# khalil-research/CaVE

Measured on NVIDIA B200. Metric: cave_loss_grad_instances_per_sec, higher is better.
Workload: dtype f64

## Files before the change

cave_b200/build.py:

```python
from __future__ import annotations

import os
import shutil
import subprocess

HERE = os.path.dirname(os.path.abspath(__file__))
CSRC = os.path.join(HERE, "csrc")
OUT_DIR = os.path.join(HERE, "_C")
LIB = os.path.join(OUT_DIR, "libcave_b200.so")
SOURCES = ["scan_kernel.cu", "solve_kernel.cu", "solve_inst_f32_f32.cu", "solve_inst_f32_f64.cu",
           "solve_inst_f64_f32.cu", "solve_inst_f64_f64.cu", "gram_kernel.cu", "dense_solve.cu", "tsp_dp.cu", "abi.cu"]
HEADERS = ["ctx.cuh", "layout.cuh", "dense.cuh", "scan_kernel.cuh", "solve_kernel.cuh", "solve_kernel_impl.cuh", "solver_core.cuh",
           os.path.join("..", "..", "include", "cave_b200.h")]
NVCC_FLAGS = ["-gencode", "arch=compute_100a,code=sm_100a", "-lineinfo", "-O3", "-std=c++17",
              "-Xcompiler", "-fPIC", "-Xptxas", "-v"]


PER_FILE_FLAGS = {"dense_solve.cu": ["-rdc=true", "-maxrregcount=128"]}


def _nvcc() -> str:
    nvcc = shutil.which("nvcc") or "/usr/local/cuda/bin/nvcc"
    if not os.path.exists(nvcc):
        raise RuntimeError("nvcc not found; cannot build the CUDA library")
    return nvcc


def is_fresh() -> bool:
    if not os.path.exists(LIB):
        return False
    t = os.path.getmtime(LIB)
    deps = [os.path.join(CSRC, s) for s in SOURCES + HEADERS] + [os.path.abspath(__file__)]
    return all(os.path.getmtime(p) <= t for p in deps)


def build(force: bool = False, verbose: bool = False, alt_name: str | None = None) -> str:
    if alt_name is None and not force and is_fresh():
        return LIB
    os.makedirs(OUT_DIR, exist_ok=True)
    objs, logs = [], []
    procs = []
    for s in SOURCES:
        obj = os.path.join(OUT_DIR, s.replace(".cu", ".o") if alt_name is None else s.replace(".cu", ".alt.o"))
        cmd = [_nvcc(), *NVCC_FLAGS, *PER_FILE_FLAGS.get(s, []), *os.environ.get("CAVE_NVCC_EXTRA", "").split(),
               "-c", os.path.join(CSRC, s), "-o", obj]
        procs.append((s, subprocess.Popen(cmd, stdout=subprocess.PIPE, stderr=subprocess.STDOUT, text=True)))
        objs.append(obj)
    for s, pr in procs:
        out, _ = pr.communicate()
        logs.append(f"== {s}\n{out}")
        if pr.returncode != 0:
            raise RuntimeError(f"nvcc failed on {s}:\n{out}")
    if alt_name is None:
        with open(os.path.join(OUT_DIR, "ptxas.log"), "w") as f:
            f.write("\n".join(logs))
    if verbose:
        print("\n".join(logs))
    target = LIB if alt_name is None else os.path.join(OUT_DIR, alt_name)
    subprocess.check_call([_nvcc(), "-gencode", "arch=compute_100a,code=sm_100a", "-shared", "-o", target, *objs,
                           "-lcudart_static", "-lpthread", "-ldl", "-lrt"])
    return target


if __name__ == "__main__":
    import sys
    alt = [a for a in sys.argv[1:] if a.endswith(".so")]
    print(build(force=True, verbose="-v" in sys.argv, alt_name=alt[0] if alt else None))
```

cave_b200/csrc/abi.cu:

```cuda
#include <cuda_runtime.h>
#include <stdarg.h>
#include <stdio.h>
#include <stdlib.h>
#include <string.h>
#include <atomic>
#include <string>

#include "../../include/cave_b200.h"
#include "layout.cuh"
#include "scan_kernel.cuh"
#include "solve_kernel.cuh"
#include "dense.cuh"

namespace cave {
size_t tsp_slot_floats(int n);
cudaError_t launch_tsp(const float* cost, int N, int n, int* tour, double* obj, void* scratch, int n_slots, cudaStream_t stream);
}

namespace {

thread_local std::string g_err;
std::atomic<unsigned long long> g_launches{0};

int fail(int code, const char* fmt, ...) {
// ... 225 lines not shown
    return pack_impl(A, m_rows, B, m_max, d, pack, pack_bytes, stream, (flags & 1) != 0);
}

int cave_pack_sparse(const int64_t* inst_off, const int64_t* row_ptr, const int32_t* col, const float* val, int64_t B,
                     int64_t m_max, int64_t d, int32_t flags, void* pack, size_t pack_bytes, void* stream) {
    if (!inst_off || !row_ptr || !col || !val) return fail(CAVE_EINVAL, "inst_off, row_ptr, col and val must not be null");
    SparseIn in;
    in.inst_off = (const long long*)inst_off; in.row_ptr = (const long long*)row_ptr; in.col = col; in.val = val;
    return pack_impl(nullptr, nullptr, B, m_max, d, pack, pack_bytes, stream, (flags & 1) != 0, &in);
}

int cave_warm_bytes(int64_t n_instances, int64_t m_max, int64_t d, size_t* out) {
    if (!out) return fail(CAVE_EINVAL, "out is null");
    if (int e = check_shape(n_instances, m_max, d)) return e;
    *out = (size_t)n_instances * cave::warm_slot_bytes(m_max);
    return CAVE_OK;
}

int cave_dense_warm_bytes(int64_t n_instances, int64_t m_max, int64_t d, size_t* out) {
    if (!out) return fail(CAVE_EINVAL, "out is null");
    if (int e = check_shape(n_instances, m_max, d)) return e;
    *out = (size_t)n_instances * cave::dense_warm_slot_bytes(m_max);
    return CAVE_OK;
}

static int forward_backward_impl(const float* A, const int32_t* m_rows, const void* pred, int64_t B, int64_t m_max, int64_t d,
                                 double sign, int mode, double inner_ratio, int reduction, int io_dtype, int compute_dtype,
                                 const cave_solver_opts* opts, void* loss, void* loss_i, void* grad, void* proj, void* rnorm,
                                 int32_t* status, int32_t* iters, void* pack, size_t pack_bytes, void* scratch,
                                 size_t scratch_bytes, void* warm, size_t warm_bytes, void* warm_dense,
                                 size_t warm_dense_bytes, const void* gram, size_t gram_bytes, void* stream) {
    const bool indexed = opts && opts->inst_index;
    if ((!A && !indexed) || !pred || !loss_i || !grad || !pack || !scratch) return fail(CAVE_EINVAL, "A, pred, loss_i, grad, pack, scratch must not be null");
    if (indexed && !opts->warm_pack) return fail(CAVE_EINVAL, "inst_index needs warm_pack (a pack built over the whole dataset)");
    if (indexed && opts->n_packed <= 0) return fail(CAVE_EINVAL, "n_packed must be positive with inst_index");
    if (int e = check_shape(B, m_max, d)) return e;
    if (mode < CAVE_MODE_EXACT || mode > CAVE_MODE_HEURISTIC) return fail(CAVE_EINVAL, "bad mode %d", mode);
    if (reduction < CAVE_REDUCE_MEAN || reduction > CAVE_REDUCE_NONE) return fail(CAVE_EINVAL, "bad reduction %d", reduction);
    if ((io_dtype != CAVE_F32 && io_dtype != CAVE_F64) || (compute_dtype != CAVE_F32 && compute_dtype != CAVE_F64))
        return fail(CAVE_EINVAL, "bad dtype (io %d, compute %d)", io_dtype, compute_dtype);
    if (!(sign == 1.0 || sign == -1.0)) return fail(CAVE_EINVAL, "sign must be +1 or -1");
    if (!(inner_ratio >= 0.0 && inner_ratio <= 1.0)) return fail(CAVE_EINVAL, "inner_ratio must be in [0, 1]");
    if (reduction != CAVE_REDUCE_NONE && !loss) return fail(CAVE_EINVAL, "loss must not be null for mean/sum");
    if (((uintptr_t)scratch & 255) != 0 || ((uintptr_t)pack & 255) != 0) return fail(CAVE_EINVAL, "pack and scratch must be 256-byte aligned");

    const int64_t Bpack = indexed ? opts->n_packed : B;
    if (int e = check_shape(Bpack, m_max, d)) return e;
    const cave::PackLayout PL = cave::make_pack_layout(Bpack, m_max, d);
    if (pack_bytes < PL.total) return fail(CAVE_ENOSPC, "pack buffer has %zu bytes, %zu needed", pack_bytes, PL.total);
    const ScratchPlan SPn = plan_scratch(opts, B, m_max, d);
    const size_t T = 8;
    const int64_t n_slots = SPn.n_slots;
    const cave::ScratchLayout SL = cave::make_scratch_layout(B, d, SPn.cr, SPn.cz, T, n_slots, SPn.n_large, SPn.large_bytes, SPn.small_bytes);
    const bool dense = dense_enabled(opts, A, m_max, d, mode);
    cave::DenseLayout DL;
    memset(&DL, 0, sizeof(DL));
    if (dense) DL = cave::make_dense_layout(B, m_max, d, dense_slots(opts, B, m_max, d), SL.total);
    const size_t need = dense ? DL.total : SL.total;
    if (scratch_bytes < need) return fail(CAVE_ENOSPC, "scratch buffer has %zu bytes, %zu needed", scratch_bytes, need);
    if (warm) {
        const size_t wneed = (size_t)Bpack * cave::warm_slot_bytes(m_max);
        if (warm_bytes < wneed) return fail(CAVE_ENOSPC, "warm-start buffer has %zu bytes, %zu needed (cave_warm_bytes of %lld instances)",
                                            warm_bytes, wneed, (long long)Bpack);
        if (((uintptr_t)warm & 15) != 0) return fail(CAVE_EINVAL, "warm-start buffer must be 16-byte aligned");
    }
    if (warm_dense) {
        const size_t wneed = (size_t)Bpack * cave::dense_warm_slot_bytes(m_max);
        if (warm_dense_bytes < wneed)
            return fail(CAVE_ENOSPC, "dense warm-start buffer has %zu bytes, %zu needed (cave_dense_warm_bytes of %lld instances)",
                        warm_dense_bytes, wneed, (long long)Bpack);
        if (((uintptr_t)warm_dense & 15) != 0) return fail(CAVE_EINVAL, "dense warm-start buffer must be 16-byte aligned");
    }
    if (gram) {
        if (!A) return fail(CAVE_EINVAL, "a Gram cache needs A (the dense path reads the rows of A)");
        if (((uintptr_t)gram & 15) != 0) return fail(CAVE_EINVAL, "Gram cache must be 16-byte aligned");
        const size_t gneed = cave::gram_cache_bytes(Bpack, 0, m_max);
        if (gram_bytes < gneed)
            return fail(CAVE_ENOSPC, "Gram cache has %zu bytes, at least %zu needed (cave_gram_cache_bytes of %lld instances)",
                        gram_bytes, gneed, (long long)Bpack);
    }

    cudaStream_t st = (cudaStream_t)stream;
    if (!(opts && opts->warm_pack)) {
        if (int e = pack_impl(A, m_rows, B, m_max, d, pack, pack_bytes, stream, env_int("CAVE_COLD_SETUP", 0) != 0, nullptr,
                              mode == CAVE_MODE_EXACT)) return e;
    }
    char* pb = (char*)pack;
    char* sb = (char*)scratch;
    cudaError_t ce = cudaMemsetAsync(sb + SL.counter, 0, 256, st);
    if (ce != cudaSuccess) return fail(CAVE_ECUDA, "cudaMemsetAsync failed: %s", cudaGetErrorString(ce));

    cave::SolveParams sp;
    memset(&sp, 0, sizeof(sp));
    sp.A = A; sp.pred = pred; sp.grad = grad; sp.proj = proj;
    sp.B = (int)B; sp.m_max = (int)m_max; sp.d = (int)d; sp.dpad = PL.dpad;
    sp.nvalid = (const int*)(pb + PL.nvalid); sp.ngen = (const int*)(pb + PL.ngen);
    sp.gennnz = (const int*)(pb + PL.gennnz); sp.nsingc = (const int*)(pb + PL.nsingc);
    sp.gen = (const int4*)(pb + PL.gen); sp.ctype = (const unsigned char*)(pb + PL.ctype); sp.avg = (const float*)(pb + PL.avg);
    sp.csr_ok = (const int*)(pb + PL.csrok); sp.maxl1 = (const float*)(pb + PL.maxl1); sp.maxl2 = (const float*)(pb + PL.maxl2);
    sp.ghash = (const ulonglong2*)(pb + PL.ghash); sp.csr_col = (const uint16_t*)(pb + PL.csr_col);
    sp.csr_val = (const float*)(pb + PL.csr_val); sp.cap_nnz = PL.cap_nnz;
    sp.counter = (int*)(sb + SL.counter); sp.loss64 = (double*)(sb + SL.loss64); sp.rnorm64 = (double*)(sb + SL.rnorm64);
    sp.status = (int*)(sb + SL.status); sp.iters = (int*)(sb + SL.iters);
    sp.slots = sb + SL.slots; sp.slot_bytes = SL.slot_bytes;
    sp.large = sb + SL.large; sp.large_bytes = SL.large_bytes; sp.n_large = (int)SL.n_large;
    sp.mode = mode; sp.inner_ratio = inner_ratio; sp.sign = sign;
    sp.gscale = reduction == CAVE_REDUCE_MEAN ? 1.0 / (double)B : 1.0;
    sp.max_iter = opts ? opts->max_iter : 0; sp.max_ls = opts ? opts->max_linesearch : 0; sp.tol = opts ? opts->tol : 0.0;
    sp.inst_index = indexed ? opts->inst_index : nullptr;
    sp.plan = (const unsigned long long*)(pb + PL.plan);
    sp.order = (indexed || env_int("CAVE_SOLVE_ORDER", 1) == 0) ? nullptr : (const int*)(pb + PL.order);
    sp.n_packed = Bpack;
    sp.setup = (((opts && opts->warm_pack) || env_int("CAVE_COLD_SETUP", 0)) && env_int("CAVE_SETUP_CACHE", 1)) ? pb + PL.setup : nullptr;
    sp.setup_stride = PL.setup_stride;
    sp.warm = (char*)warm; sp.warm_stride = (long long)cave::warm_slot_bytes(m_max); sp.warm_cap = (int)cave::warm_cap_v(m_max);
    sp.dense_flag = nullptr;
    if (dense) {
        cave::DenseParams dp;
        memset(&dp, 0, sizeof(dp));
        dp.A = A; dp.pred = pred; dp.B = (int)B; dp.m_max = (int)m_max; dp.d = (int)d;
        dp.inst_index = sp.inst_index; dp.n_packed = Bpack; dp.nvalid = sp.nvalid; dp.ngen = sp.ngen; dp.nsingc = sp.nsingc; dp.gen = sp.gen;
        dp.ctype = sp.ctype; dp.avg = sp.avg; dp.dpad = PL.dpad;
        dp.plan = (const unsigned long long*)(pb + PL.plan); dp.ws = sb; dp.L = DL; dp.force = (opts && opts->dense_mode > 0) ? 1 : 0; dp.no_handback = env_int("CAVE_DENSE_NO_HANDBACK", 0); dp.trace_b = env_int("CAVE_DENSE_TRACE", -1);
        dp.grad = grad; dp.proj = proj; dp.loss64 = sp.loss64; dp.rnorm64 = sp.rnorm64; dp.status = sp.status; dp.iters = sp.iters;
        dp.mode = mode; dp.inner_ratio = inner_ratio; dp.sign = sign; dp.gscale = sp.gscale;
        dp.max_iter = 0; dp.max_ls = sp.max_ls; dp.tol = sp.tol; dp.io_f32 = io_dtype == CAVE_F32; dp.nk = (int)(DL.d_pad / 32);
        dp.warm = (char*)warm_dense; dp.warm_stride = (long long)cave::dense_warm_slot_bytes(m_max); dp.warm_cap = (int)cave::dense_warm_cap(m_max);
        dp.gram = (const char*)gram; dp.gram_bytes = gram_bytes;
        ce = cave::launch_dense_list(dp, st);
        g_launches += 1;
        if (ce != cudaSuccess) return fail(CAVE_ECUDA, "dense list kernel launch failed: %s", cudaGetErrorString(ce));
        const int64_t rounds = (B + DL.n_slots - 1) / DL.n_slots;
        for (int64_t r = 0; r < rounds; ++r) {
            dp.round = (int)r;
            ce = cave::launch_dense_prep(dp, st);
            if (ce != cudaSuccess) return fail(CAVE_ECUDA, "dense prep kernel launch failed: %s", cudaGetErrorString(ce));
            if (!gram) {
                ce = cave::launch_dense_gram(dp, st);
                if (ce != cudaSuccess) return fail(CAVE_ECUDA, "dense Gram kernel launch failed: %s (%s)", cudaGetErrorString(ce), cave::dense_last_error());
            }
            ce = cave::launch_dense_solve(dp, st);
            g_launches += gram ? 2 : 3;
            if (ce != cudaSuccess) return fail(CAVE_ECUDA, "dense solve kernel launch failed: %s", cudaGetErrorString(ce));
        }
        sp.dense_flag = (const int*)(sb + DL.flag);
    }
    if (solve_forced()) {
        sp.smem_bytes = env_int("CAVE_SOLVE_SMEM", 110 * 1024);
        int threads = env_int("CAVE_SOLVE_THREADS", 256);
        if (threads < 32 || threads > 256 || threads % 32) threads = 256;
        sp.cfg_id = -1;
        ce = cave::launch_solve(sp, compute_dtype == CAVE_F32, io_dtype == CAVE_F32, (int)n_slots, threads, st);
        g_launches += 1;
        if (ce != cudaSuccess) return fail(CAVE_ECUDA, "solve kernel launch failed: %s", cudaGetErrorString(ce));
    } else {
        const int only = env_int("CAVE_SOLVE_CFG", -1);
        for (int i = 0; i < cave::kNumSolveConfigs; ++i) {
            const cave::SolveConfig cfg = cave::solve_config(i);
            if (only >= 0 && only < cave::kNumSolveConfigs && i != only) continue;
            int64_t grid = (int64_t)sm_count() * cfg.ctas_per_sm;
            if (grid > n_slots) grid = n_slots;
            sp.smem_bytes = cfg.smem_bytes;
            sp.cfg_id = (only >= 0 && only < cave::kNumSolveConfigs) ? -1 : i;
            ce = cave::launch_solve(sp, compute_dtype == CAVE_F32, io_dtype == CAVE_F32, (int)grid, cfg.threads, st);
            g_launches += 1;
            if (ce != cudaSuccess) return fail(CAVE_ECUDA, "solve kernel launch failed: %s", cudaGetErrorString(ce));
        }
    }

    cave::FinalizeParams fp;
    memset(&fp, 0, sizeof(fp));
    fp.B = (int)B; fp.reduction = reduction; fp.loss64 = sp.loss64; fp.rnorm64 = sp.rnorm64; fp.status = sp.status; fp.iters = sp.iters;
    fp.loss = loss; fp.loss_i = loss_i; fp.rnorm = rnorm; fp.status_out = status; fp.iters_out = iters;
    ce = cave::launch_finalize(fp, io_dtype == CAVE_F32, st);
    g_launches += 1;
    if (ce != cudaSuccess) return fail(CAVE_ECUDA, "finalize kernel launch failed: %s", cudaGetErrorString(ce));
    return CAVE_OK;
}

int cave_forward_backward(const float* A, const int32_t* m_rows, const void* pred, int64_t B, int64_t m_max, int64_t d,
                          double sign, int mode, double inner_ratio, int reduction, int io_dtype, int compute_dtype,
                          const cave_solver_opts* opts, void* loss, void* loss_i, void* grad, void* proj, void* rnorm,
                          int32_t* status, int32_t* iters, void* pack, size_t pack_bytes, void* scratch,
                          size_t scratch_bytes, void* stream) {
    return forward_backward_impl(A, m_rows, pred, B, m_max, d, sign, mode, inner_ratio, reduction, io_dtype, compute_dtype, opts,
                                 loss, loss_i, grad, proj, rnorm, status, iters, pack, pack_bytes, scratch, scratch_bytes,
                                 nullptr, 0, nullptr, 0, nullptr, 0, stream);
}

int cave_forward_backward_warm(const float* A, const int32_t* m_rows, const void* pred, int64_t B, int64_t m_max, int64_t d,
                               double sign, int mode, double inner_ratio, int reduction, int io_dtype, int compute_dtype,
                               const cave_solver_opts* opts, void* loss, void* loss_i, void* grad, void* proj, void* rnorm,
                               int32_t* status, int32_t* iters, void* pack, size_t pack_bytes, void* scratch,
                               size_t scratch_bytes, void* warm, size_t warm_bytes, void* stream) {
    if (!warm) return fail(CAVE_EINVAL, "warm must not be null (use cave_forward_backward for a call without warm-start state)");
    if (!(opts && opts->warm_pack))
// ... 193 lines not shown
```

cave_b200/csrc/scan_kernel.cu:

```cuda
#include <cuda_runtime.h>
#include <stdint.h>
#include <stdlib.h>
#include "layout.cuh"
#include "scan_kernel.cuh"

namespace cave {

__device__ __forceinline__ uint32_t smem_u32(const void* p) { return (uint32_t)__cvta_generic_to_shared(p); }

__device__ __forceinline__ void mbar_init(uint64_t* bar, uint32_t count) {
    asm volatile("mbarrier.init.shared::cta.b64 [%0], %1;" ::"r"(smem_u32(bar)), "r"(count));
}
__device__ __forceinline__ void mbar_expect_tx(uint64_t* bar, uint32_t bytes) {
    asm volatile("mbarrier.arrive.expect_tx.shared::cta.b64 _, [%0], %1;" ::"r"(smem_u32(bar)), "r"(bytes) : "memory");
}
__device__ __forceinline__ void mbar_wait(uint64_t* bar, uint32_t parity) {
    asm volatile(
        "{\n"
        ".reg .pred p;\n"
        "WAIT_LOOP:\n"
        "mbarrier.try_wait.parity.shared::cta.b64 p, [%0], %1;\n"
        "@p bra DONE;\n"
        "bra WAIT_LOOP;\n"
        "DONE:\n"
        "}\n" ::"r"(smem_u32(bar)), "r"(parity) : "memory");
}
__device__ __forceinline__ void tma_bulk_g2s(void* dst, const void* src, uint32_t bytes, uint64_t* bar) {
    asm volatile("cp.async.bulk.shared::cluster.global.mbarrier::complete_tx::bytes [%0], [%1], %2, [%3];" ::"r"(
                     smem_u32(dst)),
                 "l"(src), "r"(bytes), "r"(smem_u32(bar))
                 : "memory");
}

__device__ __forceinline__ uint64_t mix64d(uint64_t x) {
    x ^= x >> 33; x *= 0xff51afd7ed558ccdULL; x ^= x >> 33; x *= 0xc4ceb9fe1a85ec53ULL; x ^= x >> 33;
    return x;
}

struct RowAcc {
    float l1, l2, lv;
    int lk, n;
    __device__ __forceinline__ void add(float v, int k) {
        l1 += fabsf(v);
        l2 = fmaf(v, v, l2);
        lk = k; lv = v; ++n;
    }
};

template <int NT>
__global__ void __launch_bounds__(NT) scan_kernel(ScanParams p) {
    extern __shared__ __align__(128) unsigned char smem[];
    const int tid = threadIdx.x, lane = tid & 31, warp = tid >> 5;
    constexpr int NW = NT / 32;
    const int d = p.d, R = p.R, S = p.stages;
    const int b = blockIdx.x;

    unsigned char* ring = smem;
    float* avg_gen = (float*)(smem + (size_t)S * p.stage_stride);
    int* sing = (int*)(avg_gen + d);
    uint64_t* full = (uint64_t*)align_up((size_t)(sing + d), 8);
    float* r_l1 = (float*)(full + S);
    float* r_nrm = r_l1 + R;
    float* r_inv = r_nrm + R;
    float* r_val = r_inv + R;
    int* r_cnt = (int*)(r_val + R);
    int* r_k = r_cnt + R;
    int* s_cnt = r_k + R;
    unsigned char* ctype = (unsigned char*)align_up((size_t)(s_cnt + 8), 16);

    const int m_b = p.m_rows ? min(max(p.m_rows[b], 0), p.m_max) : p.m_max;
    const int ntiles = (m_b + R - 1) / R;
    const float* A_b = p.A + (size_t)b * p.m_max * d;

    for (int k = tid; k < d; k += NT) { avg_gen[k] = 0.f; sing[k] = 0; }
    for (int k = tid; k < (int)p.dpad; k += NT) ctype[k] = 0;
    if (tid < 8) s_cnt[tid] = 0;
    if (tid == 0) {
        for (int s = 0; s < S; ++s) mbar_init(full + s, 1);
        asm volatile("fence.mbarrier_init.release.cluster;" ::: "memory");
    }
    __syncthreads();

    auto issue = [&](int t) {
        const int s = t % S;
        const int rows = min(R, m_b - t * R);
        const uintptr_t a = (uintptr_t)(A_b + (size_t)t * R * d);
        const uintptr_t a0 = a & ~(uintptr_t)15;
// ... 687 lines not shown
        p.nvalid[b] = s_cnt[0]; p.navg[b] = s_cnt[1]; p.ngen[b] = s_cnt[2]; p.gennnz[b] = s_cnt[3]; p.nsingc[b] = s_cnt[4];
        p.csr_ok[b] = s_cnt[6] ? 0 : (s_cnt[7] ? 1 : 3);
        p.maxl1[b] = m1; p.maxl2[b] = m2;
    }
}

cudaError_t launch_scan_sparse(const ScanParams& pk, const long long* inst_off, const long long* row_ptr, const int* col,
                               const float* val, cudaStream_t stream) {
    SparseScanParams q;
    q.inst_off = inst_off; q.row_ptr = row_ptr; q.col = col; q.val = val; q.pk = pk;
    const size_t smem = sparse_scan_smem_bytes(pk.d, pk.m_max, pk.dpad);
    if (smem > 220 * 1024) return cudaErrorInvalidValue;
    if (smem > 48 * 1024) {
        cudaError_t e = cudaFuncSetAttribute(scan_sparse_kernel, cudaFuncAttributeMaxDynamicSharedMemorySize, (int)smem);
        if (e != cudaSuccess) return e;
    }
    scan_sparse_kernel<<<dim3((unsigned)pk.B), dim3(kSparseThreads), smem, stream>>>(q);
    return cudaGetLastError();
}

constexpr int kPlanMaxRows = 512;
__global__ void __launch_bounds__(256) plan_kernel(PlanParams p) {
    __shared__ unsigned long long hp[8][kPlanMaxRows];
    const int lane = threadIdx.x & 31, w = threadIdx.x >> 5;
    const int b = blockIdx.x * 8 + w;
    if (b >= p.B) return;
    const int ngen = p.ngen[b], nnz = p.gennnz[b], ok = p.csr_ok[b];
    const bool dense_path = p.nsingc[b] == 0;
    int paired = 0;
    if (ngen > 0 && !dense_path && (ok & 1) && ngen <= kPlanMaxRows) {
        const int4* gen = p.gen4 + (size_t)b * p.m_max;
        const ulonglong2* gh = p.ghash + (size_t)b * p.m_max;
        unsigned long long want[kPlanMaxRows / 32];
#pragma unroll
        for (int u = 0; u < kPlanMaxRows / 32; ++u) {
            const int i = u * 32 + lane;
            want[u] = 0;
            if (i < ngen) { const ulonglong2 h = gh[gen[i].x]; hp[w][i] = h.x; want[u] = h.y; }
        }
        __syncwarp();
#pragma unroll
        for (int u = 0; u < kPlanMaxRows / 32; ++u) {
            const int i = u * 32 + lane;
            if (u * 32 < ngen) {
                bool hit = false;
                for (int j = 0; j < ngen; ++j) hit |= (j != i) & (hp[w][j] == want[u]);
                paired += (i < ngen && hit) ? 1 : 0;
            }
        }
        for (int o = 16; o > 0; o >>= 1) paired += __shfl_xor_sync(0xffffffffu, paired, o);
    }
    if (lane == 0) {
        const int nv = ngen - paired / 2;
        const long long nnz_kept = ngen > 0 ? (long long)nnz * nv / ngen : 0;
        const bool skip = p.nvalid[b] == 0;
        size_t hot8, work8, hot4, work4;
        instance_footprint(p.d, skip ? 0 : ngen, nv, nnz_kept, (ok & 3) == 3, dense_path, 8, &hot8, &work8);
        instance_footprint(p.d, skip ? 0 : ngen, nv, nnz_kept, (ok & 3) == 3, dense_path, 4, &hot4, &work4);
        long long key = skip ? 0 : (dense_path ? (long long)ngen * p.d : nnz_kept + 16ll * nv);
        p.okey[b] = (int)(key > 0x7fffffffll ? 0x7fffffffll : key);
        atomicAdd(p.plan + PLAN_N, 1ull);
        atomicAdd(p.plan + PLAN_SUM8, (unsigned long long)work8);
        atomicAdd(p.plan + PLAN_SUM4, (unsigned long long)work4);
        atomicMax(p.plan + PLAN_MAXHOT8, (unsigned long long)hot8);
        atomicMax(p.plan + PLAN_MAXHOT4, (unsigned long long)hot4);
    }
}

__global__ void __launch_bounds__(256) order_kernel(PlanParams p) {
    const int lane = threadIdx.x & 31;
    const int b = blockIdx.x * 8 + (threadIdx.x >> 5);
    if (b >= p.B) return;
    if (p.B > kOrderMaxBatch) { if (lane == 0) p.order[b] = b; return; }
    const int mine = p.okey[b];
    int rank = 0;
    for (int j = lane; j < p.B; j += 32) {
        const int k = p.okey[j];
        rank += (k > mine) | ((k == mine) & (j < b));
    }
    for (int o = 16; o > 0; o >>= 1) rank += __shfl_xor_sync(0xffffffffu, rank, o);
    if (lane == 0) p.order[rank] = b;
}

constexpr int kSetupThreads = 128;
__host__ __device__ inline size_t setup_smem_bytes(int64_t cap_v, int64_t d) {
    return (size_t)cap_v * (8 + 8 + 4 + 4 + 4 + 4 + 1) + 64 + (size_t)(d + 2) * 8 + 64;
}
__global__ void __launch_bounds__(kSetupThreads) setup_kernel(PlanParams p, int enabled) {
    extern __shared__ __align__(16) char ssm[];
    __shared__ int s_nv, s_nz;
    const int b = blockIdx.x;
    const int tid = threadIdx.x, lane = tid & 31, warp = tid >> 5;
    constexpr int NW = kSetupThreads / 32;
    char* blk = p.setup + (size_t)b * p.setup_stride;
    int* hdr = (int*)blk;
    const int mB = p.ngen[b], d = p.d;
    const bool eligible = enabled && p.nsingc[b] > 0 && mB > 0 && (p.csr_ok[b] & 3) == 3 && mB <= p.setup_cap_v && p.nvalid[b] > 0;
    if (!eligible) { if (tid == 0) hdr[0] = 0; return; }
    const SetupBlock SB = make_setup_block(p.setup_cap_v, p.cap_nnz, d);
    const int cv = (int)p.setup_cap_v;
    unsigned long long* hpos = (unsigned long long*)ssm;
    unsigned long long* hneg = hpos + cv;
    int* goff = (int*)(hneg + cv);
    int* gcnt = goff + cv + 1;
    int* cand = gcnt + cv + 1;
    int* keep = cand + cv + 2;
    int* cnt = keep + cv + 1;
    int* cur = cnt + d + 2;
    unsigned char* rtype = (unsigned char*)(cur + d + 1);
    const int4* gen = p.gen4 + (size_t)b * p.m_max;
    const ulonglong2* gh = p.ghash + (size_t)b * p.m_max;
    const uint16_t* pcol = p.csr_col + (size_t)b * p.cap_nnz;
    const float* pval = p.csr_val + (size_t)b * p.cap_nnz;
    for (int i = tid; i < mB; i += kSetupThreads) {
        const int4 g = gen[i]; gcnt[i] = g.y; goff[i] = g.z;
        const ulonglong2 h = gh[g.x]; hpos[i] = h.x; hneg[i] = h.y;
    }
    for (int k = tid; k <= d + 1; k += kSetupThreads) cnt[k] = 0;
    __syncthreads();
    for (int i = warp; i < mB; i += NW) {
        const int pi = goff[i], ni = gcnt[i];
        const unsigned long long want = hneg[i];
        int c0 = -1;
        for (int j0 = 0; j0 < mB && c0 < 0; j0 += 32) {
            const int j = j0 + lane;
            const bool hit = j < mB && j != i && hpos[j] == want && gcnt[j] == ni;
            unsigned m = __ballot_sync(0xffffffffu, hit);
            while (m && c0 < 0) {
                const int jj = j0 + __ffs(m) - 1;
                const int pj = goff[jj];
                bool ok = true;
                for (int e = lane; e < ni; e += 32) ok = ok & (pcol[pi + e] == pcol[pj + e]) & (pval[pi + e] == -pval[pj + e]);
                if (!__ballot_sync(0xffffffffu, !ok)) c0 = jj;
                m &= m - 1;
            }
        }
        if (lane == 0) cand[i] = c0;
    }
    __syncthreads();
    for (int i = tid; i < mB; i += kSetupThreads) {
        const int j = cand[i];
        rtype[i] = (j >= 0 && cand[j] == i) ? (i < j ? 1 : 2) : 0;
    }
    __syncthreads();
    unsigned char* o_vfree = (unsigned char*)(blk + SB.vfree);
    int* o_rptr = (int*)(blk + SB.rptr);
    int* o_cptr = (int*)(blk + SB.cptr);
    uint16_t* o_rcol = (uint16_t*)(blk + SB.rcol);
    uint16_t* o_crow = (uint16_t*)(blk + SB.crow);
    signed char* o_rval = (signed char*)(blk + SB.rval);
    signed char* o_cval = (signed char*)(blk + SB.cval);
    int* rp = cand;
    if (warp == 0) {
        int nvb = 0, run = 0;
        for (int i0 = 0; i0 < mB; i0 += 32) {
            const int i = i0 + lane;
            const bool kp = i < mB && rtype[i] != 2;
            const unsigned m = __ballot_sync(0xffffffffu, kp);
            int len = kp ? gcnt[i] : 0, incl = len;
#pragma unroll
            for (int o = 1; o < 32; o <<= 1) { const int u = __shfl_up_sync(0xffffffffu, incl, o); if (lane >= o) incl += u; }
            if (kp) {
                const int v = nvb + __popc(m & ((1u << lane) - 1u));
                keep[v] = i; o_vfree[v] = (unsigned char)(rtype[i] == 1);
                const int start = run + incl - len;
                rp[v] = start; o_rptr[v] = start;
            }
            nvb += __popc(m);
            run += __shfl_sync(0xffffffffu, incl, 31);
        }
        if (lane == 0) { rp[nvb] = run; o_rptr[nvb] = run; s_nv = nvb; s_nz = run; }
    }
    __syncthreads();
    const int nv = s_nv, nz = s_nz;
    for (int v = warp; v < nv; v += NW) {
        const int src = goff[keep[v]], dst = rp[v], n = rp[v + 1] - dst;
        for (int e = lane; e < n; e += 32) {
            const uint16_t c = pcol[src + e];
            o_rcol[dst + e] = c; o_rval[dst + e] = (signed char)pval[src + e];
            atomicAdd(&cnt[c + 1], 1);
        }
    }
    __syncthreads();
    if (warp == 0) {
        int carry = 0;
        for (int k0 = 1; k0 <= d; k0 += 32) {
            const int k = k0 + lane;
            int v = k <= d ? cnt[k] : 0;
#pragma unroll
            for (int o = 1; o < 32; o <<= 1) { const int u = __shfl_up_sync(0xffffffffu, v, o); if (lane >= o) v += u; }
            v += carry;
            if (k <= d) cnt[k] = v;
            carry = __shfl_sync(0xffffffffu, v, 31);
        }
    }
    __syncthreads();
    for (int k = tid; k <= d; k += kSetupThreads) { o_cptr[k] = cnt[k]; if (k < d) cur[k] = cnt[k]; }
    __syncthreads();
    {
        const int c_lo = (int)(((long long)d * warp) / NW), c_hi = (int)(((long long)d * (warp + 1)) / NW);
        constexpr int U = 8;
        int cc[U]; float vv[U];
        auto fetch = [&](int v) {
            const int src = goff[keep[v]], n = rp[v + 1] - rp[v];
#pragma unroll
            for (int u = 0; u < U; ++u) {
                const int e = lane + 32 * u;
                cc[u] = e < n ? (int)pcol[src + e] : -1;
                vv[u] = e < n ? pval[src + e] : 0.f;
            }
        };
        if (nv > 0) fetch(0);
        for (int v = 0; v < nv; ++v) {
            int c0[U]; float v0[U];
#pragma unroll
            for (int u = 0; u < U; ++u) { c0[u] = cc[u]; v0[u] = vv[u]; }
            const int n = rp[v + 1] - rp[v];
            if (v + 1 < nv) fetch(v + 1);
#pragma unroll
            for (int u = 0; u < U; ++u) {
                if (c0[u] >= c_lo && c0[u] < c_hi) {
                    const int q = cur[c0[u]]; cur[c0[u]] = q + 1;
                    o_crow[q] = (uint16_t)v; o_cval[q] = (signed char)v0[u];
                }
            }
            if (n > 32 * U) {
                const int src = goff[keep[v]];
                for (int e = 32 * U + lane; e < n; e += 32) {
                    const int c = pcol[src + e];
                    if (c >= c_lo && c < c_hi) { const int q = cur[c]; cur[c] = q + 1; o_crow[q] = (uint16_t)v; o_cval[q] = (signed char)pval[src + e]; }
                }
            }
            __syncwarp();
        }
    }
    if (tid == 0) {
        hdr[1] = nv; hdr[2] = nz;
        hdr[3] = (int)SB.vfree; hdr[4] = (int)SB.rptr; hdr[5] = (int)SB.cptr; hdr[6] = (int)SB.rcol; hdr[7] = (int)SB.crow;
        hdr[8] = (int)SB.rval; hdr[9] = (int)SB.cval;
        hdr[0] = 1;
    }
}

__global__ void clear_setup_kernel(char* setup, long long stride, int B) {
    const int b = blockIdx.x * blockDim.x + threadIdx.x;
    if (b < B) *(int*)(setup + (size_t)b * (size_t)stride) = 0;
}
cudaError_t launch_clear_setup(char* setup, long long stride, int B, cudaStream_t stream) {
    clear_setup_kernel<<<(unsigned)((B + 255) / 256), 256, 0, stream>>>(setup, stride, B);
    return cudaGetLastError();
}

cudaError_t launch_plan(const PlanParams& p, cudaStream_t stream) {
    plan_kernel<<<dim3((unsigned)((p.B + 7) / 8)), dim3(256), 0, stream>>>(p);
    cudaError_t e = cudaGetLastError();
    if (e != cudaSuccess) return e;
    order_kernel<<<dim3((unsigned)((p.B + 7) / 8)), dim3(256), 0, stream>>>(p);
    e = cudaGetLastError();
    if (e != cudaSuccess || !p.setup) return e;
    const size_t smem = setup_smem_bytes(p.setup_cap_v, p.d);
    const char* off = getenv("CAVE_SETUP_CACHE");
    const int enabled = (smem <= 200 * 1024 && !(off && off[0] == '0')) ? 1 : 0;
    const size_t use = enabled ? smem : 0;
    if (use > 48 * 1024) {
        e = cudaFuncSetAttribute(setup_kernel, cudaFuncAttributeMaxDynamicSharedMemorySize, (int)use);
        if (e != cudaSuccess) return e;
    }
    setup_kernel<<<dim3((unsigned)p.B), dim3(kSetupThreads), use, stream>>>(p, enabled);
    return cudaGetLastError();
}

}
```

cave_b200/qpsolver.py:

```python
from __future__ import annotations

import ctypes
import os
from dataclasses import dataclass

import torch

from . import _lib

_PRECISIONS = {"fp64": _lib.F64, "float64": _lib.F64, "double": _lib.F64,
               "fp32": _lib.F32, "float32": _lib.F32, "single": _lib.F32}


_DENSE = {"auto": 0, None: 0, True: 1, False: -1, "on": 1, "off": -1}


def _opts(max_iter=None, max_linesearch=None, tol=None, cap_rows=None, cap_nnz=None, warm=False,
          index=None, n_packed=0, dense="auto", dense_slots=None) -> _lib.SolverOpts:
    if dense not in _DENSE:
        raise ValueError("dense must be 'auto', True or False")
    return _lib.SolverOpts(int(max_iter or 0), int(max_linesearch or 0), float(tol or 0.0),
                           int(cap_rows or 0), int(cap_nnz or 0), int(bool(warm)), _DENSE[dense],
                           index.data_ptr() if index is not None else None, int(n_packed), int(dense_slots or 0))

# ... 129 lines not shown
        A = tight_ctrs.detach().cpu().numpy()
        B, m, d = A.shape
        inst_off, row_ptr, cols, vals = [0], [0], [], []
        for b in range(B):
            keep = np.flatnonzero(np.abs(A[b]).sum(axis=1) > 0)
            for r in keep:
                k = np.flatnonzero(A[b, r])
                cols.append(k.astype(np.int32)); vals.append(A[b, r, k].astype(np.float32))
                row_ptr.append(row_ptr[-1] + len(k))
            inst_off.append(inst_off[-1] + len(keep))
        return SparseConstraints(torch.tensor(inst_off, dtype=torch.int64), torch.tensor(row_ptr, dtype=torch.int64),
                                 torch.from_numpy(np.concatenate(cols) if cols else np.zeros(0, np.int32)),
                                 torch.from_numpy(np.concatenate(vals) if vals else np.zeros(0, np.float32)), m, d)

    @staticmethod
    def from_instances(insts, m_max: int | None = None) -> "SparseConstraints":
        import numpy as np
        d = insts[0].d
        m_max = max(i.m for i in insts) if m_max is None else m_max
        inst_off = np.zeros(len(insts) + 1, np.int64)
        ptrs, cols, vals = [np.zeros(1, np.int64)], [], []
        base = 0
        for b, it in enumerate(insts):
            order = np.lexsort((it.cols, it.rows))
            cnt = np.bincount(it.rows, minlength=it.m).astype(np.int64)
            ptrs.append(base + np.cumsum(cnt)); base += int(cnt.sum())
            cols.append(it.cols[order].astype(np.int32)); vals.append(it.vals[order].astype(np.float32))
            inst_off[b + 1] = inst_off[b] + it.m
        return SparseConstraints(torch.from_numpy(inst_off), torch.from_numpy(np.concatenate(ptrs)),
                                 torch.from_numpy(np.concatenate(cols)), torch.from_numpy(np.concatenate(vals)), int(m_max), int(d))

    def pin_memory(self) -> "SparseConstraints":
        return SparseConstraints(self.inst_off.pin_memory(), self.row_ptr.pin_memory(), self.col.pin_memory(), self.val.pin_memory(),
                                 self.m_max, self.d)


def pack_constraints_sparse(sc: SparseConstraints, device=None, cache_setup: bool = True,
                            warm_start: bool = False) -> CavePack:
    lib = _lib.load()
    dev = _device_of(sc.val, device)
    B, m, d = sc.batch, int(sc.m_max), int(sc.d)
    io = _to_device(sc.inst_off, dev, torch.int64)
    rp = _to_device(sc.row_ptr, dev, torch.int64)
    col = _to_device(sc.col, dev, torch.int32)
    val = _to_device(sc.val, dev, torch.float32)
    nbytes = ctypes.c_size_t()
    _lib.check(lib.cave_pack_bytes(B, m, d, ctypes.byref(nbytes)))
    buf = torch.empty(nbytes.value, dtype=torch.uint8, device=dev)
    with torch.cuda.device(dev):
        stream = torch.cuda.current_stream(dev).cuda_stream
        _lib.check(lib.cave_pack_sparse(_ptr(io), _ptr(rp), _ptr(col), _ptr(val), B, m, d, 1 if cache_setup else 0,
                                        _ptr(buf), nbytes.value, ctypes.c_void_p(stream)))
    warm = _warm_buffer(lib.cave_warm_bytes, B, m, d, dev) if warm_start else None
    return CavePack(buf, (B, m, d), 0, None, 0, warm)


def _call_forward_backward(lib, pack: CavePack | None, *args) -> None:
    if pack is not None and pack.gram is not None:
        *head, stream = args
        nwarm = pack.warm.numel() if pack.warm is not None else 0
        ndense = pack.warm_dense.numel() if pack.warm_dense is not None else 0
        _lib.check(lib.cave_forward_backward_resident(*head, _ptr(pack.warm), nwarm, _ptr(pack.warm_dense), ndense,
                                                      _ptr(pack.gram), pack.gram.numel(), stream))
    elif pack is not None and pack.warm_dense is not None:
        *head, stream = args
        nwarm = pack.warm.numel() if pack.warm is not None else 0
        _lib.check(lib.cave_forward_backward_warm_ex(*head, _ptr(pack.warm), nwarm, _ptr(pack.warm_dense),
                                                     pack.warm_dense.numel(), stream))
    elif pack is not None and pack.warm is not None:
        *head, stream = args
        _lib.check(lib.cave_forward_backward_warm(*head, _ptr(pack.warm), pack.warm.numel(), stream))
    else:
        _lib.check(lib.cave_forward_backward(*args))


def cave_forward_backward(pred_cost: torch.Tensor, tight_ctrs: torch.Tensor, sign: float, mode: int,
                          inner_ratio: float = 0.2, reduction: str = "mean", precision: str = "fp64",
                          want_proj: bool = False, want_status: bool = False, pack: CavePack | None = None,
                          index: torch.Tensor | None = None,
                          m_rows: torch.Tensor | None = None, device=None, max_iter=None, max_linesearch=None,
                          tol=None, cap_rows=None, cap_nnz=None, dense="auto", dense_slots=None) -> dict:
    lib = _lib.load()
    if isinstance(tight_ctrs, SparseConstraints):
        pack = pack_constraints_sparse(tight_ctrs, device=device, cache_setup=False)
        tight_ctrs = None
    if index is None and tight_ctrs is None and pack is not None and pack.shape[0] == pred_cost.shape[0]:
        index = torch.arange(pred_cost.shape[0], dtype=torch.int32, device=pack.buf.device)
    if index is not None:
        return _forward_backward_indexed(lib, pred_cost, tight_ctrs, sign, mode, inner_ratio, reduction, precision,
                                         want_proj, want_status, pack, index, device, max_iter, max_linesearch, tol,
                                         cap_rows, cap_nnz, dense, dense_slots)
    if pred_cost.dim() != 2 or tight_ctrs.dim() != 3 or tight_ctrs.shape[0] != pred_cost.shape[0] \
            or tight_ctrs.shape[2] != pred_cost.shape[1]:
        raise ValueError(f"shape mismatch: pred_cost {tuple(pred_cost.shape)}, tight_ctrs {tuple(tight_ctrs.shape)}")
    if reduction not in _lib.REDUCE:
        raise ValueError(f"No reduction '{reduction}'.")
    if precision not in _PRECISIONS:
        raise ValueError(f"precision must be one of {sorted(_PRECISIONS)}")
    dev = _device_of(tight_ctrs if tight_ctrs.is_cuda else pred_cost, device)
    io_dtype = torch.float64 if pred_cost.dtype == torch.float64 else torch.float32
    pred = _to_device(pred_cost.detach(), dev, io_dtype)
    A = _to_device(tight_ctrs.detach(), dev, torch.float32)
    B, m, d = A.shape
    if B == 0:
        z = torch.zeros((), dtype=io_dtype, device=dev)
        return dict(loss=z if reduction != "none" else torch.zeros(0, dtype=io_dtype, device=dev),
                    loss_i=torch.zeros(0, dtype=io_dtype, device=dev), grad=torch.zeros_like(pred))
    if m == 0:
        A = torch.zeros((B, 1, d), dtype=torch.float32, device=dev)
        m = 1
    compute = _PRECISIONS[precision]
    opts = _opts(max_iter, max_linesearch, tol, cap_rows, cap_nnz, warm=pack is not None, dense=dense, dense_slots=dense_slots)
    nb = ctypes.c_size_t()
    if pack is not None:
        if pack.shape != (B, m, d) or pack.buf.device != dev or pack.data_ptr != A.data_ptr() \
                or pack.version != int(tight_ctrs._version):
            raise ValueError("pack does not belong to this tight_ctrs tensor (other storage, shape or device, or the "
                             "tensor was modified in place after pack_constraints); for batches drawn from a dataset "
                             "pack the whole dataset once and pass index=")
        pack_buf = pack.buf
    else:
        _lib.check(lib.cave_pack_bytes(B, m, d, ctypes.byref(nb)))
        pack_buf = torch.empty(nb.value, dtype=torch.uint8, device=dev)
    _lib.check(lib.cave_scratch_bytes(B, m, d, compute, ctypes.byref(opts), ctypes.byref(nb)))
    scratch = torch.empty(nb.value, dtype=torch.uint8, device=dev)
    loss = torch.empty((), dtype=io_dtype, device=dev)
    loss_i = torch.empty(B, dtype=io_dtype, device=dev)
    grad = torch.empty((B, d), dtype=io_dtype, device=dev)
    proj = torch.empty((B, d), dtype=io_dtype, device=dev) if want_proj else None
    rnorm = torch.empty(B, dtype=io_dtype, device=dev) if (want_proj or want_status) else None
    status = torch.empty(B, dtype=torch.int32, device=dev) if want_status else None
    iters = torch.empty(B, dtype=torch.int32, device=dev) if want_status else None
    if m_rows is not None:
        m_rows = _to_device(m_rows, dev, torch.int32)
    with torch.cuda.device(dev):
        stream = torch.cuda.current_stream(dev).cuda_stream
        _call_forward_backward(
            lib, pack, _ptr(A), _ptr(m_rows), _ptr(pred), B, m, d, float(sign), int(mode), float(inner_ratio),
            _lib.REDUCE[reduction], _lib.F64 if io_dtype == torch.float64 else _lib.F32, compute,
            ctypes.byref(opts), _ptr(loss), _ptr(loss_i), _ptr(grad), _ptr(proj), _ptr(rnorm), _ptr(status),
            _ptr(iters), _ptr(pack_buf), pack_buf.numel(), _ptr(scratch), scratch.numel(), ctypes.c_void_p(stream))
    out = dict(loss=loss_i if reduction == "none" else loss, loss_i=loss_i, grad=grad)
    if want_proj:
        out["proj"], out["rnorm"] = proj, rnorm
    if want_status:
        out["status"], out["iters"], out["rnorm"] = status, iters, rnorm
    if os.environ.get("CAVE_KEEP_SCRATCH"):
        out["_scratch"], out["_opts"] = scratch, opts
    return out


def _forward_backward_indexed(lib, pred_cost, ctrs, sign, mode, inner_ratio, reduction, precision, want_proj,
                              want_status, pack, index, device, max_iter, max_linesearch, tol, cap_rows, cap_nnz,
                              dense="auto", dense_slots=None) -> dict:
    if pack is None:
        raise ValueError("index= needs pack= (pack_constraints over the whole dataset)")
    if reduction not in _lib.REDUCE:
        raise ValueError(f"No reduction '{reduction}'.")
    if precision not in _PRECISIONS:
        raise ValueError(f"precision must be one of {sorted(_PRECISIONS)}")
    dev = pack.buf.device
    N, m, d = pack.shape
    if pred_cost.dim() != 2 or pred_cost.shape[1] != d or index.dim() != 1 or index.shape[0] != pred_cost.shape[0]:
        raise ValueError(f"shape mismatch: pred_cost {tuple(pred_cost.shape)}, index {tuple(index.shape)}, pack {pack.shape}")
    io_dtype = torch.float64 if pred_cost.dtype == torch.float64 else torch.float32
    pred = _to_device(pred_cost.detach(), dev, io_dtype)
    idx = _to_device(index.detach(), dev, torch.int32)
# ... 63 lines not shown
```

Measured before the change: 509,300.

## Enable cold setup cache by default and stage CSR in shared memory

Turns on the per-instance setup (CSC transpose) stage by default on cold calls and for sparse constraints. The setup kernel now stages small CSR columns/values into shared memory as int8, and builds the transpose with an atomic bucket scatter plus per-column insertion sort of packed keys. It also adds a parallel first-candidate prefilter for hash matching, a multi-warp prefix scan, and 256 threads per block. The aim is to cut setup-kernel latency so the cached transposed layout speeds the solver, at the cost of extra work on every cold call. The int8 cast assumes constraint values are small integers.

```diff
diff --git a/cave_b200/build.py b/cave_b200/build.py
--- a/cave_b200/build.py
+++ b/cave_b200/build.py
@@ -10,7 +10,7 @@
 LIB = os.path.join(OUT_DIR, "libcave_b200.so")
 SOURCES = ["scan_kernel.cu", "solve_kernel.cu", "solve_inst_f32_f32.cu", "solve_inst_f32_f64.cu",
            "solve_inst_f64_f32.cu", "solve_inst_f64_f64.cu", "gram_kernel.cu", "dense_solve.cu", "tsp_dp.cu", "abi.cu"]
-HEADERS = ["ctx.cuh", "layout.cuh", "dense.cuh", "scan_kernel.cuh", "solve_kernel.cuh", "solve_kernel_impl.cuh", "solver_core.cuh",
+HEADERS = ["ctx.cuh", "layout.cuh", "setup_stage.cuh", "dense.cuh", "scan_kernel.cuh", "solve_kernel.cuh", "solve_kernel_impl.cuh", "solver_core.cuh",
            os.path.join("..", "..", "include", "cave_b200.h")]
 NVCC_FLAGS = ["-gencode", "arch=compute_100a,code=sm_100a", "-lineinfo", "-O3", "-std=c++17",
               "-Xcompiler", "-fPIC", "-Xptxas", "-v"]
diff --git a/cave_b200/csrc/abi.cu b/cave_b200/csrc/abi.cu
--- a/cave_b200/csrc/abi.cu
+++ b/cave_b200/csrc/abi.cu
@@ -331,7 +331,7 @@
 
     cudaStream_t st = (cudaStream_t)stream;
     if (!(opts && opts->warm_pack)) {
-        if (int e = pack_impl(A, m_rows, B, m_max, d, pack, pack_bytes, stream, env_int("CAVE_COLD_SETUP", 0) != 0, nullptr,
+        if (int e = pack_impl(A, m_rows, B, m_max, d, pack, pack_bytes, stream, env_int("CAVE_COLD_SETUP", 1) != 0, nullptr,
                               mode == CAVE_MODE_EXACT)) return e;
     }
     char* pb = (char*)pack;
@@ -360,7 +360,7 @@
     sp.plan = (const unsigned long long*)(pb + PL.plan);
     sp.order = (indexed || env_int("CAVE_SOLVE_ORDER", 1) == 0) ? nullptr : (const int*)(pb + PL.order);
     sp.n_packed = Bpack;
-    sp.setup = (((opts && opts->warm_pack) || env_int("CAVE_COLD_SETUP", 0)) && env_int("CAVE_SETUP_CACHE", 1)) ? pb + PL.setup : nullptr;
+    sp.setup = (((opts && opts->warm_pack) || env_int("CAVE_COLD_SETUP", 1)) && env_int("CAVE_SETUP_CACHE", 1)) ? pb + PL.setup : nullptr;
     sp.setup_stride = PL.setup_stride;
     sp.warm = (char*)warm; sp.warm_stride = (long long)cave::warm_slot_bytes(m_max); sp.warm_cap = (int)cave::warm_cap_v(m_max);
     sp.dense_flag = nullptr;
diff --git a/cave_b200/csrc/scan_kernel.cu b/cave_b200/csrc/scan_kernel.cu
--- a/cave_b200/csrc/scan_kernel.cu
+++ b/cave_b200/csrc/scan_kernel.cu
@@ -3,6 +3,7 @@
 #include <stdlib.h>
 #include "layout.cuh"
 #include "scan_kernel.cuh"
+#include "setup_stage.cuh"
 
 namespace cave {
 
@@ -856,21 +857,14 @@
     if (lane == 0) p.order[rank] = b;
 }
 
-constexpr int kSetupThreads = 128;
-__host__ __device__ inline size_t setup_smem_bytes(int64_t cap_v, int64_t d) {
-    return (size_t)cap_v * (8 + 8 + 4 + 4 + 4 + 4 + 1) + 64 + (size_t)(d + 2) * 8 + 64;
-}
-__global__ void __launch_bounds__(kSetupThreads) setup_kernel(PlanParams p, int enabled) {
-    extern __shared__ __align__(16) char ssm[];
-    __shared__ int s_nv, s_nz;
-    const int b = blockIdx.x;
+template <typename V>
+__device__ __forceinline__ void setup_instance(const PlanParams& p, int b, char* ssm, const uint16_t* pcol, const V* pval,
+                                               int& s_nv, int& s_nz) {
     const int tid = threadIdx.x, lane = tid & 31, warp = tid >> 5;
     constexpr int NW = kSetupThreads / 32;
     char* blk = p.setup + (size_t)b * p.setup_stride;
     int* hdr = (int*)blk;
     const int mB = p.ngen[b], d = p.d;
-    const bool eligible = enabled && p.nsingc[b] > 0 && mB > 0 && (p.csr_ok[b] & 3) == 3 && mB <= p.setup_cap_v && p.nvalid[b] > 0;
-    if (!eligible) { if (tid == 0) hdr[0] = 0; return; }
     const SetupBlock SB = make_setup_block(p.setup_cap_v, p.cap_nnz, d);
     const int cv = (int)p.setup_cap_v;
     unsigned long long* hpos = (unsigned long long*)ssm;
@@ -880,25 +874,31 @@
     int* cand = gcnt + cv + 1;
     int* keep = cand + cv + 2;
     int* cnt = keep + cv + 1;
-    int* cur = cnt + d + 2;
-    unsigned char* rtype = (unsigned char*)(cur + d + 1);
+    unsigned char* rtype = (unsigned char*)(cnt + d + 2);
     const int4* gen = p.gen4 + (size_t)b * p.m_max;
     const ulonglong2* gh = p.ghash + (size_t)b * p.m_max;
-    const uint16_t* pcol = p.csr_col + (size_t)b * p.cap_nnz;
-    const float* pval = p.csr_val + (size_t)b * p.cap_nnz;
     for (int i = tid; i < mB; i += kSetupThreads) {
         const int4 g = gen[i]; gcnt[i] = g.y; goff[i] = g.z;
         const ulonglong2 h = gh[g.x]; hpos[i] = h.x; hneg[i] = h.y;
     }
     for (int k = tid; k <= d + 1; k += kSetupThreads) cnt[k] = 0;
     __syncthreads();
+    for (int i = tid; i < mB; i += kSetupThreads) {
+        const unsigned long long want = hneg[i];
+        const int ni = gcnt[i];
+        int f = -1;
+#pragma unroll 4
+        for (int j = mB - 1; j >= 0; --j) f = (j != i && hpos[j] == want && gcnt[j] == ni) ? j : f;
+        cand[i] = f;
+    }
+    __syncthreads();
     for (int i = warp; i < mB; i += NW) {
-        const int pi = goff[i], ni = gcnt[i];
+        const int pi = goff[i], ni = gcnt[i], first = cand[i];
         const unsigned long long want = hneg[i];
         int c0 = -1;
-        for (int j0 = 0; j0 < mB && c0 < 0; j0 += 32) {
+        for (int j0 = first & ~31; first >= 0 && j0 < mB && c0 < 0; j0 += 32) {
             const int j = j0 + lane;
-            const bool hit = j < mB && j != i && hpos[j] == want && gcnt[j] == ni;
+            const bool hit = j >= first && j < mB && j != i && hpos[j] == want && gcnt[j] == ni;
             unsigned m = __ballot_sync(0xffffffffu, hit);
             while (m && c0 < 0) {
                 const int jj = j0 + __ffs(m) - 1;
@@ -909,6 +909,7 @@
                 m &= m - 1;
             }
         }
+        __syncwarp();
         if (lane == 0) cand[i] = c0;
     }
     __syncthreads();
@@ -956,37 +957,67 @@
         }
     }
     __syncthreads();
-    if (warp == 0) {
+    {
+        __shared__ int s_wsum[NW];
+        const int per = (d + NW - 1) / NW, k_lo = 1 + warp * per, k_hi = min(d, k_lo + per - 1);
         int carry = 0;
-        for (int k0 = 1; k0 <= d; k0 += 32) {
+        for (int k0 = k_lo; k0 <= k_hi; k0 += 32) {
             const int k = k0 + lane;
-            int v = k <= d ? cnt[k] : 0;
+            int v = k <= k_hi ? cnt[k] : 0;
 #pragma unroll
             for (int o = 1; o < 32; o <<= 1) { const int u = __shfl_up_sync(0xffffffffu, v, o); if (lane >= o) v += u; }
             v += carry;
-            if (k <= d) cnt[k] = v;
+            if (k <= k_hi) cnt[k] = v;
             carry = __shfl_sync(0xffffffffu, v, 31);
         }
-    }
-    __syncthreads();
-    for (int k = tid; k <= d; k += kSetupThreads) { o_cptr[k] = cnt[k]; if (k < d) cur[k] = cnt[k]; }
-    __syncthreads();
-    {
+        if (lane == 0) s_wsum[warp] = carry;
+        __syncthreads();
+        int off = 0;
+        for (int w = 0; w < warp; ++w) off += s_wsum[w];
+        for (int k = k_lo + lane; k <= k_hi; k += 32) cnt[k] += off;
+    }
+    __syncthreads();
+    for (int k = tid; k <= d; k += kSetupThreads) o_cptr[k] = cnt[k];
+    __syncthreads();
+    if constexpr (sizeof(V) == 1) {
+        uint16_t* key = (uint16_t*)(((uintptr_t)(rtype + cv) + 15) & ~(uintptr_t)15);
+        for (int v = warp; v < nv; v += NW) {
+            const int src = goff[keep[v]], n = rp[v + 1] - rp[v];
+            for (int e = lane; e < n; e += 32)
+                key[atomicAdd(&cnt[pcol[src + e]], 1)] = (uint16_t)((v << 8) | (unsigned char)pval[src + e]);
+        }
+        __syncthreads();
+        for (int c = tid; c < d; c += kSetupThreads) {
+            const int lo = c > 0 ? cnt[c - 1] : 0, hi = cnt[c];
+            for (int i = lo + 1; i < hi; ++i) {
+                const uint16_t k = key[i];
+                int j = i - 1;
+                while (j >= lo && key[j] > k) { key[j + 1] = key[j]; --j; }
+                key[j + 1] = k;
+            }
+        }
+        __syncthreads();
+        for (int q = tid; q < nz; q += kSetupThreads) {
+            const uint16_t k = key[q];
+            o_crow[q] = (uint16_t)(k >> 8); o_cval[q] = (signed char)(k & 0xff);
+        }
+    } else {
+        int* cur = cnt;
         const int c_lo = (int)(((long long)d * warp) / NW), c_hi = (int)(((long long)d * (warp + 1)) / NW);
         constexpr int U = 8;
-        int cc[U]; float vv[U];
+        int cc[U]; V vv[U];
         auto fetch = [&](int v) {
             const int src = goff[keep[v]], n = rp[v + 1] - rp[v];
 #pragma unroll
             for (int u = 0; u < U; ++u) {
                 const int e = lane + 32 * u;
                 cc[u] = e < n ? (int)pcol[src + e] : -1;
-                vv[u] = e < n ? pval[src + e] : 0.f;
+                vv[u] = e < n ? pval[src + e] : V(0);
             }
         };
         if (nv > 0) fetch(0);
         for (int v = 0; v < nv; ++v) {
-            int c0[U]; float v0[U];
+            int c0[U]; V v0[U];
 #pragma unroll
             for (int u = 0; u < U; ++u) { c0[u] = cc[u]; v0[u] = vv[u]; }
             const int n = rp[v + 1] - rp[v];
@@ -1013,6 +1044,34 @@
         hdr[3] = (int)SB.vfree; hdr[4] = (int)SB.rptr; hdr[5] = (int)SB.cptr; hdr[6] = (int)SB.rcol; hdr[7] = (int)SB.crow;
         hdr[8] = (int)SB.rval; hdr[9] = (int)SB.cval;
         hdr[0] = 1;
+    }
+}
+
+__global__ void __launch_bounds__(kSetupThreads, 3) setup_kernel(PlanParams p, int enabled) {
+    extern __shared__ __align__(16) char ssm[];
+    __shared__ int s_nv, s_nz;
+    const int b = blockIdx.x, tid = threadIdx.x;
+    const int mB = p.ngen[b];
+    const bool eligible = enabled && p.nsingc[b] > 0 && mB > 0 && (p.csr_ok[b] & 3) == 3 && mB <= p.setup_cap_v && p.nvalid[b] > 0;
+    if (!eligible) { if (tid == 0) *(int*)(p.setup + (size_t)b * p.setup_stride) = 0; return; }
+    const int stage = (int)setup_stage_nnz(p.cap_nnz), nnz = p.gennnz[b];
+    const uint16_t* pcol = p.csr_col + (size_t)b * p.cap_nnz;
+    const float* pval = p.csr_val + (size_t)b * p.cap_nnz;
+    if (nnz <= stage) {
+        uint16_t* s_col = (uint16_t*)ssm;
+        signed char* s_val = (signed char*)(ssm + (size_t)stage * 2);
+        const uint4* c16 = (const uint4*)pcol;
+        const float4* v16 = (const float4*)pval;
+#pragma unroll 8
+        for (int k = tid; k < (nnz + 7) / 8; k += kSetupThreads) ((uint4*)s_col)[k] = c16[k];
+#pragma unroll 8
+        for (int k = tid; k < (nnz + 3) / 4; k += kSetupThreads) {
+            const float4 f = v16[k];
+            ((char4*)s_val)[k] = make_char4((signed char)f.x, (signed char)f.y, (signed char)f.z, (signed char)f.w);
+        }
+        setup_instance<signed char>(p, b, ssm + (size_t)stage * 3, s_col, s_val, s_nv, s_nz);
+    } else {
+        setup_instance<float>(p, b, ssm + (size_t)stage * 3, pcol, pval, s_nv, s_nz);
     }
 }
 
@@ -1032,7 +1091,7 @@
     order_kernel<<<dim3((unsigned)((p.B + 7) / 8)), dim3(256), 0, stream>>>(p);
     e = cudaGetLastError();
     if (e != cudaSuccess || !p.setup) return e;
-    const size_t smem = setup_smem_bytes(p.setup_cap_v, p.d);
+    const size_t smem = setup_smem_bytes(p.setup_cap_v, p.cap_nnz, p.d);
     const char* off = getenv("CAVE_SETUP_CACHE");
     const int enabled = (smem <= 200 * 1024 && !(off && off[0] == '0')) ? 1 : 0;
     const size_t use = enabled ? smem : 0;
diff --git a/cave_b200/csrc/setup_stage.cuh b/cave_b200/csrc/setup_stage.cuh
--- /dev/null
+++ b/cave_b200/csrc/setup_stage.cuh
@@ -0,0 +1,16 @@
+#pragma once
+#include "layout.cuh"
+
+namespace cave {
+
+constexpr int kSetupThreads = 256;
+constexpr int64_t kSetupStageNnz = 12288;
+CAVE_HD int64_t setup_stage_nnz(int64_t cap_nnz) {
+    const int64_t c = (int64_t)align_up((size_t)cap_nnz, 16);
+    return c < kSetupStageNnz ? c : kSetupStageNnz;
+}
+CAVE_HD size_t setup_smem_bytes(int64_t cap_v, int64_t cap_nnz, int64_t d) {
+    return (size_t)setup_stage_nnz(cap_nnz) * 5 + (size_t)cap_v * (8 + 8 + 4 + 4 + 4 + 4 + 1) + 64 + (size_t)(d + 2) * 4 + 64 + 16;
+}
+
+}
diff --git a/cave_b200/qpsolver.py b/cave_b200/qpsolver.py
--- a/cave_b200/qpsolver.py
+++ b/cave_b200/qpsolver.py
@@ -235,7 +235,7 @@
                           tol=None, cap_rows=None, cap_nnz=None, dense="auto", dense_slots=None) -> dict:
     lib = _lib.load()
     if isinstance(tight_ctrs, SparseConstraints):
-        pack = pack_constraints_sparse(tight_ctrs, device=device, cache_setup=False)
+        pack = pack_constraints_sparse(tight_ctrs, device=device)
         tight_ctrs = None
     if index is None and tight_ctrs is None and pack is not None and pack.shape[0] == pred_cost.shape[0]:
         index = torch.arange(pred_cost.shape[0], dtype=torch.int32, device=pack.buf.device)
```

After: 520,300 (median of 6 runs). +2.2%, better.
